# haskoin/haskoin-node

Measured on AMD Instinct MI355X. Metric: ECDSA verifies/sec (1/8 GPU) + verdict mismatches vs libsecp256k1, higher is better.
Workload: dtype u32 (256-bit integer limbs)

## Files before the change

haskoin-node_amd/csrc/hkv_group.h:

```cpp
#pragma once
#include "hkv_scalar.h"

namespace hkv {

struct ge { fe x, y; };
struct gej { fe x, y, z; };


__constant__ static const uint32_t FE_GX[8] = {0x16F81798u, 0x59F2815Bu, 0x2DCE28D9u, 0x029BFCDBu,
                                               0xCE870B07u, 0x55A06295u, 0xF9DCBBACu, 0x79BE667Eu};
__constant__ static const uint32_t FE_GY[8] = {0xFB10D4B8u, 0x9C47D08Fu, 0xA6855419u, 0xFD17B448u,
                                               0x0E1108A8u, 0x5DA4FBFCu, 0x26A3C465u, 0x483ADA77u};
__constant__ static const uint32_t FE_BETA[8] = {0x719501EEu, 0xC1396C28u, 0x12F58995u, 0x9CF04975u,
                                                 0xAC3434E9u, 0x6E64479Eu, 0x657C0710u, 0x7AE96A2Bu};

HKV_DEV void ge_set_g(ge& r) {
#pragma unroll
  for (int i = 0; i < 8; ++i) { r.x.v[i] = FE_GX[i]; r.y.v[i] = FE_GY[i]; }
}
HKV_DEV void gej_set_ge(gej& r, const ge& a) {
  r.x = a.x;
  r.y = a.y;
  fe_set_u32(r.z, 1);
}
HKV_DEV void gej_cmov(gej& r, const gej& a, bool f) {
  fe_cmov(r.x, a.x, f);
  fe_cmov(r.y, a.y, f);
  fe_cmov(r.z, a.z, f);
}

template <bool FC = false>
HKV_DEV void gej_double(gej& r, const gej& a) {
  fe A, B, M, E, t, u;
  fe_sqr<FC>(A, a.x);
  fe_sqr<FC>(B, a.y);
  fe_mul<FC>(M, a.x, B);
  fe_mul_small(E, A, 3);
  fe_half(E, E);
  fe_mul<FC>(r.z, a.y, a.z);
  fe_sqr<FC>(t, E);
  fe_shl(u, M, 1);
  fe_sub(r.x, t, u);
  fe_sub(t, r.x, M);
  fe_sqrmul_sum<FC>(t, B, E, t);
  fe_neg_compl(r.y, t);
}

template <bool FC = false>
HKV_DEV void gej_add_tail(gej& r, const gej& a, const fe& h, const fe& rr) {
  fe hh, hhh, v, t, t2;
  fe_sqr<FC>(hh, h);
  fe_mul<FC>(hhh, h, hh);
  fe_mul<FC>(v, a.x, hh);
  fe_mul<FC>(r.z, a.z, h);
  fe_sqr<FC>(t, rr);
  fe_sub(t, t, hhh);
  fe_shl(t2, v, 1);
  fe_sub(r.x, t, t2);
  fe_sub(v, r.x, v);
  fe_mul_sum<FC>(v, rr, v, a.y, hhh);
  fe_neg_compl(r.y, v);
}

template <bool FC = false>
HKV_DEV void gej_add_ge_core(gej& r, const gej& a, const fe& az, const fe& bx, const fe& by,
                             bool& hz, bool& rz, fe* zr) {
  fe z2, u2, s2, h, rr, t;
  fe_sqr<FC>(z2, az);
  fe_mul<FC>(u2, bx, z2);
  fe_mul<FC>(t, az, z2);
  fe_mul<FC>(s2, by, t);
  fe_sub(h, u2, a.x);
  fe_sub(rr, s2, a.y);
  hz = fe_is_zero(h);
  rz = fe_is_zero(rr);
  gej_add_tail<FC>(r, a, h, rr);
  if (zr) *zr = h;
}

template <bool FC = false>
HKV_DEV void gej_accumulate(gej& acc, bool& inf, const fe& az, const fe& tx, const fe& ty, bool take) {
  fe h, rr;
  {
    fe z2, t;
    fe_sqr<FC>(z2, az);
    fe_mul<FC>(h, tx, z2);
    fe_mul<FC>(t, az, z2);
    fe_mul<FC>(rr, ty, t);
  }
  fe_sub(h, h, acc.x);
  fe_sub(rr, rr, acc.y);
  const bool live = take && !inf;
  const bool hz = fe_is_zero(h);
  if (live && !hz) gej_add_tail<FC>(acc, acc, h, rr);
  const bool degen = live && hz;
  if (__builtin_expect(__any(degen), 0)) {
    const bool rz = fe_is_zero(rr);
    if (degen && rz) gej_double<FC>(acc, acc);
    inf = inf || (degen && !rz);
  }
}
HKV_DEV void gej_double_ilp(gej& r, const gej& a) {
  fe A, B, M, Z3, C, E, t;
  fe_sqr2(A, a.x, B, a.y);
  fe_mul2(M, a.x, B, Z3, a.y, a.z);
  fe_mul_small(E, A, 3);
  fe_half(E, E);
  fe_sqr2(C, B, t, E);
  r.z = Z3;
  fe_shl(B, M, 1);
  fe_sub(r.x, t, B);
  fe_sub(t, M, r.x);
  fe_mul(t, E, t);
  fe_sub(r.y, t, C);
}

HKV_DEV void gej_accumulate_ilp(gej& acc, bool& inf, const fe& az, const fe& tx, const fe& ty, bool take) {
  fe h, rr, hh;
  {
    fe z2, t;
    fe_sqr(z2, az);
    fe_mul2(h, tx, z2, t, az, z2);
    fe_sub(h, h, acc.x);
    fe_sqrmul(hh, h, rr, ty, t);
  }
  fe_sub(rr, rr, acc.y);
  const bool live = take && !inf;
  const bool hz = fe_is_zero(h);
  if (live && !hz) {
    fe hhh, v, r2, z3, t2;
    fe_mul2(hhh, h, hh, v, acc.x, hh);
    fe_sqrmul(r2, rr, z3, acc.z, h);
    acc.z = z3;
    fe_sub(r2, r2, hhh);
    fe_shl(t2, v, 1);
    fe_sub(acc.x, r2, t2);
    fe_sub(v, v, acc.x);
    fe_mul2(v, rr, v, hhh, acc.y, hhh);
    fe_sub(acc.y, v, hhh);
  }
  const bool degen = live && hz;
  if (__builtin_expect(__any(degen), 0)) {
    const bool rz = fe_is_zero(rr);
    if (degen && rz) gej_double(acc, acc);
    inf = inf || (degen && !rz);
  }
}

HKV_DEV uint32_t dpp_xch(uint32_t v) {
  return (uint32_t)__builtin_amdgcn_mov_dpp((int)v, 0xB1, 0xF, 0xF, false);
}
HKV_DEV uint32_t dpp_bc1(uint32_t v) {
  return (uint32_t)__builtin_amdgcn_mov_dpp((int)v, 0xF5, 0xF, 0xF, false);
}
HKV_DEV uint32_t dpp_bc0(uint32_t v) {
  return (uint32_t)__builtin_amdgcn_mov_dpp((int)v, 0xA0, 0xF, 0xF, false);
}
HKV_DEV void fe_xch(fe& r, const fe& a) {
#pragma unroll
  for (int i = 0; i < 8; ++i) r.v[i] = dpp_xch(a.v[i]);
}
HKV_DEV void fe_bc1(fe& r, const fe& a) {
#pragma unroll
  for (int i = 0; i < 8; ++i) r.v[i] = dpp_bc1(a.v[i]);
}
HKV_DEV void fe_sel(fe& r, const fe& a, const fe& b, uint32_t odd) {
#pragma unroll
  for (int i = 0; i < 8; ++i) r.v[i] = (a.v[i] & ~odd) | (b.v[i] & odd);
}
HKV_DEV bool pair_even(bool f) { return dpp_bc0(f ? 1u : 0u) != 0; }
HKV_DEV bool pair_odd(bool f) { return dpp_bc1(f ? 1u : 0u) != 0; }

HKV_DEV void pair_double(fe& P, fe& Z, uint32_t odd) {
  fe R1, T, O1, R2, R3, P1, P2, r, Q, t;
  fe_sqr(R1, P);
  fe_xch(T, R1);
  fe_sel(O1, T, Z, odd);
  fe_mul(R2, P, O1);
  fe_sqr(R3, T);
  fe_sel(P2, R2, R3, odd);
  fe_xch(P1, P2);
  fe_sel(O1, R3, R2, odd);
  fe_lin2(r, P1, odd ? 36u : 9u, P2, odd ? 27u : 8u);
  fe_shl_var(Q, O1, odd ? 1u : 3u);
  fe_xch(O1, Q);
  fe_cneg(O1, O1, odd != 0);
  fe_mul_add(t, T, r, O1);
  fe_sel(P, r, t, odd);
  Z = Q;
}

HKV_DEV void pair_add_tail(fe& P, fe& Z, const fe& H, const fe& R3, const fe& Rr, uint32_t odd) {
  fe O1, O2, R5, R6, W, X3, D, R7, t;
  fe_sel(O1, H, Rr, odd);
  fe_sel(O2, R3, Rr, odd);
  fe_mul(R5, O1, O2);
  fe_xch(t, H);
  fe_sel(O1, P, Z, odd);
  fe_sel(O2, R3, t, odd);
  fe_mul(R6, O1, O2);
  fe_xch(W, R5);
  fe_sub(X3, W, R5);
  fe_shl(t, R6, 1);
  fe_sub(X3, X3, t);
  fe_sub(D, R6, X3);
  fe_xch(t, D);
  fe_xch(O1, P);
  fe_sel(O1, O1, Rr, odd);
  fe_sel(O2, R5, t, odd);
  fe_mul(R7, O1, O2);
  fe_xch(t, R7);
  fe_sub(t, R7, t);
  fe_sel(P, X3, t, odd);
  Z = R6;
}

HKV_DEV void pair_accumulate(fe& P, fe& Z, bool& inf, const fe& TXY, bool take, uint32_t odd) {
  fe z2, O1, O2, R2, H, R3, Rr;
  fe_sqr(z2, Z);
  fe_bc1(O2, z2);
  fe_sel(O1, TXY, Z, odd);
  fe_mul(R2, O1, O2);
  fe_sub(H, R2, P);
  fe_sel(O1, H, TXY, odd);
  fe_sel(O2, H, R2, odd);
  fe_mul(R3, O1, O2);
  fe_sub(Rr, R3, P);
  const bool live = take && !inf;
  const bool hz = pair_even(fe_is_zero(H));
  if (live && !hz) pair_add_tail(P, Z, H, R3, Rr, odd);
// ... 135 lines not shown
```

haskoin-node_amd/csrc/hkv_kernels.hip:

```cpp
#include "hkv_group.h"
#include "hkv_hash.h"
#include "hkv_layout.h"
#include "hkv_joint_digits.h"
#include "hkv_internal.h"
#include "hkv_sighash_dev.h"
#include "hkv_tail_plan.h"

namespace hkv {

HKV_DEV uint32_t rec_word_at(const uint32_t* w, int off) {
  const int k = off >> 2, s = off & 3;
  if (s == 0) return w[k];
  return __builtin_amdgcn_alignbyte(w[k + 1], w[k], s);
}
HKV_DEV void rec_be256(uint32_t out[8], const uint32_t* w, int off) {
#pragma unroll
  for (int j = 0; j < 8; ++j) out[7 - j] = __builtin_bswap32(rec_word_at(w, off + 4 * j));
}

__constant__ static const uint32_t PMN[8] = {0x2FC9BAEEu, 0x402DA172u, 0x50B75FC4u, 0x45512319u, 1u, 0, 0, 0};

template <class W>
struct SoA {
  W* p;
// ... 361 lines not shown
}

struct StdArgs {
  const uint8_t* txs;
  uint32_t n_tx;
  const uint32_t* txt;
  const uint8_t* scripts;
  uint32_t scripts_len;
  const hkv_input_job* jobs;
  int32_t forkid;
  uint32_t* ms_desc;
  uint64_t* ms_off;
  unsigned long long* ms_ctr;
  const uint32_t* tx_off;
};
HKV_DEV void std_lane_prologue(uint32_t i, uint32_t n, SoAView iv, const StdArgs& sa);

HKV_DEV uint4* qtab_ptr(uint32_t* qs, uint32_t n_lanes, uint32_t lane, int entry, int c) {
  return reinterpret_cast<uint4*>(qs) + ((size_t)entry * n_lanes + lane) * QTAB_QUADS_PER_ENTRY + c;
}
HKV_DEV void qtab_store(uint32_t* __restrict__ qs, uint32_t n_lanes, uint32_t lane, int entry, int c, const fe& a) {
  uint4* p = qtab_ptr(qs, n_lanes, lane, entry, c);
  p[0] = make_uint4(a.v[0], a.v[1], a.v[2], a.v[3]);
  p[1] = make_uint4(a.v[4], a.v[5], a.v[6], a.v[7]);
}
HKV_DEV void qtab_load(const uint32_t* __restrict__ qs, uint32_t n_lanes, uint32_t lane, int entry, int c, fe& a) {
  const uint4* p = qtab_ptr(const_cast<uint32_t*>(qs), n_lanes, lane, entry, c);
  const uint4 v0 = p[0], v1 = p[1];
  a.v[0] = v0.x; a.v[1] = v0.y; a.v[2] = v0.z; a.v[3] = v0.w;
  a.v[4] = v1.x; a.v[5] = v1.y; a.v[6] = v1.z; a.v[7] = v1.w;
}

template <bool ILP>
HKV_DEV void ec_double(gej& acc) {
  if constexpr (ILP) gej_double_ilp(acc, acc);
  else gej_double<true>(acc, acc);
}
template <bool ILP>
HKV_DEV void ec_accumulate(gej& acc, bool& inf, const fe& az, const fe& tx, const fe& ty, bool take) {
  if constexpr (ILP) gej_accumulate_ilp(acc, inf, az, tx, ty, take);
  else gej_accumulate<true>(acc, inf, az, tx, ty, take);
}

template <bool ILP = false>
HKV_DEV void gsum_lane(SoACView iv, const uint32_t* __restrict__ gtab, uint32_t i, bool valid, gej& A, bool& ainf);
HKV_DEV void gej_add_var(gej& acc, bool& inf, const gej& b, bool binf);
HKV_DEV bool x_matches_r(const fe& Xin, const fe& Z, const uint32_t r[8]);

HKV_DEV void lane_q(ge& q, SoACView iv, uint32_t i, bool valid) {
  fe x, w;
#pragma unroll
  for (int k = 0; k < 8; ++k) {
    x.v[k] = iv.get(IM_QX, k, i);
    w.v[k] = iv.get(IM_W, k, i);
  }
  fe_mul(q.x, x, w);
  fe_sqr(q.y, w);
  if (!valid) ge_set_g(q);
}

HKV_DEV void qtable_build(const ge& q, uint32_t* __restrict__ qs, uint32_t n_lanes, uint32_t lane, fe& Zg) {
  gej p2, pj;
  gej_set_ge(p2, q);
  gej_double(p2, p2);
  fe z2, qx, qy;
  fe_sqr(z2, p2.z);
  fe_mul(qx, q.x, z2);
  fe_mul(z2, z2, p2.z);
  fe_mul(qy, q.y, z2);
  qtab_store(qs, n_lanes, lane, 0, 0, qx);
  qtab_store(qs, n_lanes, lane, 0, 2, qy);
  qtab_store(qs, n_lanes, lane, 1, 0, p2.x);
  qtab_store(qs, n_lanes, lane, 1, 2, p2.y);
  pj.x = p2.x;
  pj.y = p2.y;
  fe_set_u32(pj.z, 1);
#pragma unroll 1
  for (int j = 2; j < QTAB_ENTRIES; ++j) {
    bool hz, rz;
    fe h;
    gej_add_ge_core(pj, pj, pj.z, qx, qy, hz, rz, &h);
    qtab_store(qs, n_lanes, lane, j, 0, pj.x);
    qtab_store(qs, n_lanes, lane, j, 2, pj.y);
    qtab_store(qs, n_lanes, lane, (j - 1), 4, h);
  }
  fe_mul(Zg, p2.z, pj.z);
  fe beta;
#pragma unroll
  for (int k = 0; k < 8; ++k) beta.v[k] = FE_BETA[k];
  {
    fe bx;
    fe_mul(bx, pj.x, beta);
    qtab_store(qs, n_lanes, lane, QTAB_ENTRIES - 1, 4, bx);
  }
  fe rho;
  fe_set_u32(rho, 1);
#pragma unroll 1
  for (int j = QTAB_ENTRIES - 2; j >= 0; --j) {
    fe x, y, t;
    if (j >= 1) {
      qtab_load(qs, n_lanes, lane, j, 4, t);
      fe_mul(rho, rho, t);
    }
    qtab_load(qs, n_lanes, lane, j, 0, x);
    qtab_load(qs, n_lanes, lane, j, 2, y);
    fe_sqr(t, rho);
    fe_mul(x, x, t);
    fe_mul(t, t, rho);
    fe_mul(y, y, t);
    qtab_store(qs, n_lanes, lane, j, 0, x);
    qtab_store(qs, n_lanes, lane, j, 2, y);
    fe_mul(x, x, beta);
    qtab_store(qs, n_lanes, lane, j, 4, x);
  }
}

typedef uint32_t JqLds[4][8][WG];
HKV_DEV uint4* jq_ptr(uint32_t* qs, uint32_t n_lanes, uint32_t lane, int entry, int c) {
  return reinterpret_cast<uint4*>(qs) + ((size_t)entry * n_lanes + lane) * JQ_QUADS_PER_ENTRY + c;
}
HKV_DEV void quads_store(uint4* p, const fe& a) {
  p[0] = make_uint4(a.v[0], a.v[1], a.v[2], a.v[3]);
  p[1] = make_uint4(a.v[4], a.v[5], a.v[6], a.v[7]);
}
HKV_DEV void quads_load(const uint4* p, fe& a) {
  const uint4 v0 = p[0], v1 = p[1];
  a.v[0] = v0.x; a.v[1] = v0.y; a.v[2] = v0.z; a.v[3] = v0.w;
  a.v[4] = v1.x; a.v[5] = v1.y; a.v[6] = v1.z; a.v[7] = v1.w;
}
HKV_DEV void jq_load(const uint32_t* __restrict__ qs, uint32_t n_lanes, uint32_t lane, int entry, int c, fe& a) {
  quads_load(jq_ptr(const_cast<uint32_t*>(qs), n_lanes, lane, entry, c), a);
}
struct JqPark {
  JqLds* lds;
  uint4 *spare, *zslot, *last;
  HKV_DEV uint4* quads(int h) const { return h < 6 ? spare + 2 * (h - 4) : h == 6 ? zslot : last + 2 * (h - 7); }
  HKV_DEV void store(int h, const fe& a) const {
    if (h < 4) {
#pragma unroll
      for (int k = 0; k < 8; ++k) (*lds)[h][k][threadIdx.x] = a.v[k];
    } else {
      quads_store(quads(h), a);
    }
  }
  HKV_DEV void load(int h, fe& a) const {
    if (h < 4) {
#pragma unroll
      for (int k = 0; k < 8; ++k) a.v[k] = (*lds)[h][k][threadIdx.x];
    } else {
      quads_load(quads(h), a);
    }
  }
};
HKV_DEV void qtable_build_joint(const ge& q, uint32_t* __restrict__ qs, uint32_t n_lanes, uint32_t lane, uint4* zslot,
                                JqLds* lds, fe& Zg) {
  static_assert(JD_ENTRIES == JQ_ENTRIES, "one entry per orbit");
  const JqPark park = {lds, reinterpret_cast<uint4*>(qs) + (size_t)JQ_ENTRIES * JQ_QUADS_PER_ENTRY * n_lanes +
                                (size_t)lane * JQ_SPARE_QUADS,
                       zslot, jq_ptr(qs, n_lanes, lane, JQ_ENTRIES - 1, 0)};
  gej p2, pj;
  gej_set_ge(p2, q);
  gej_double(p2, p2);
  {
    fe z2, qx, qy;
    fe_sqr(z2, p2.z);
    fe_mul(qx, q.x, z2);
    fe_mul(z2, z2, p2.z);
    fe_mul(qy, q.y, z2);
    quads_store(jq_ptr(qs, n_lanes, lane, 0, 0), qx);
    quads_store(jq_ptr(qs, n_lanes, lane, 0, 2), qy);
  }
  quads_store(jq_ptr(qs, n_lanes, lane, 1, 0), p2.x);
  quads_store(jq_ptr(qs, n_lanes, lane, 1, 2), p2.y);
  pj.x = p2.x;
  pj.y = p2.y;
  fe_set_u32(pj.z, 1);
#pragma unroll 1
  for (int j = 2; j < JQ_ENTRIES; ++j) {
    const uint32_t e = (JD_STEP_E >> (2 * (j - 1))) & 3u;
    const bool neg = ((JD_STEP_S >> (j - 1)) & 1u) != 0;
    bool hz, rz;
    fe h, tx, ty;
    jq_load(qs, n_lanes, lane, 0, 0, tx);
    if (e != 0u) {
      fe beta, bx;
#pragma unroll
      for (int k = 0; k < 8; ++k) beta.v[k] = FE_BETA[k];
      fe_mul(bx, tx, beta);
      if (e == 2u) {
        fe_add(bx, tx, bx);
        fe_neg(bx, bx);
      }
      tx = bx;
    }
    jq_load(qs, n_lanes, lane, 0, 2, ty);
    fe_cneg(ty, ty, neg);
    gej_add_ge_core(pj, pj, pj.z, tx, ty, hz, rz, &h);
    if (j < JQ_ENTRIES - 1) {
      quads_store(jq_ptr(qs, n_lanes, lane, j, 0), pj.x);
      quads_store(jq_ptr(qs, n_lanes, lane, j, 2), pj.y);
    }
    park.store(j - 2, h);
  }
  fe_mul(Zg, p2.z, pj.z);
  fe rho;
  fe_set_u32(rho, 1);
#pragma unroll 1
  for (int j = JQ_ENTRIES - 2; j >= 0; --j) {
    fe x, y, t;
    if (j >= 1) {
      park.load(j - 1, t);
      fe_mul(rho, rho, t);
    }
    jq_load(qs, n_lanes, lane, j, 0, x);
    jq_load(qs, n_lanes, lane, j, 2, y);
    fe_sqr(t, rho);
    fe_mul(x, x, t);
    fe_mul(t, t, rho);
    fe_mul(y, y, t);
    quads_store(jq_ptr(qs, n_lanes, lane, j, 0), x);
    quads_store(jq_ptr(qs, n_lanes, lane, j, 2), y);
  }
  quads_store(park.last, pj.x);
  quads_store(park.last + 2, pj.y);
}

template <bool ILP>
HKV_DEV void q_chain(gej& acc, bool& inf, SoACView iv, uint32_t i, bool valid, const uint32_t* __restrict__ qs,
                     uint32_t n_lanes, uint32_t lane, const uint32_t& signs) {
  inf = true;
  fe_set_zero(acc.x);
  fe_set_zero(acc.y);
  fe_set_zero(acc.z);
  uint32_t dw = valid ? iv.get(IM_DIG, NWIN - 1, i) : DIG_ZERO;
  int win = NWIN - 1;
  bool dbl = false;
  int x1 = 0, x2 = 0;
  int nterm = 2;
  {
    const uint32_t dw2 = valid ? iv.get(IM_DIG, NWIN - 2, i) : DIG_ZERO;
    const int t1 = (((int)(dw & QDIG_MASK) - QBIAS) << QW) + (int)(dw2 & QDIG_MASK) - QBIAS;
    const int t2 = (((int)((dw >> QDIG_BITS) & QDIG_MASK) - QBIAS) << QW) + (int)((dw2 >> QDIG_BITS) & QDIG_MASK) - QBIAS;
    if (!__any(t1 < 0 || t1 > 2 * QBIAS || t2 < 0 || t2 > 2 * QBIAS)) {
      const int e1 = t1 < QBIAS ? t1 : QBIAS, e2 = t2 < QBIAS ? t2 : QBIAS;
      x1 = t1 - e1;
      x2 = t2 - e2;
      dw = (uint32_t)(e1 + QBIAS) | ((uint32_t)(e2 + QBIAS) << QDIG_BITS);
      win = NWIN - 2;
      nterm = 4;
    }
  }
#pragma unroll 1
  for (; win >= 0; --win) {
    const int d1 = (int)(dw & QDIG_MASK) - QBIAS, d2 = (int)((dw >> QDIG_BITS) & QDIG_MASK) - QBIAS;
    const uint32_t dw_next = (win > 0 && valid) ? iv.get(IM_DIG, win - 1, i) : DIG_ZERO;
    if (dbl) {
#pragma unroll 1
      for (int d = 0; d < QW; ++d) {
        if (!inf) ec_double<ILP>(acc);
      }
    }
    dbl = true;
#pragma unroll 1
    for (int t = 0; t < nterm; ++t) {
      const int slot = t & 1;
      const int dg = t < 2 ? (slot == 0 ? d1 : d2) : (slot == 0 ? x1 : x2);
      const bool take = dg != 0;
      if (t >= 2 && !__any(take)) continue;
      const int mg = dg < 0 ? -dg : dg;
      const int ie = mg ? mg - 1 : 0;
      const bool neg = (dg < 0) != (((signs >> slot) & 1u) != 0);
      fe tx, ty;
      qtab_load(qs, n_lanes, lane, ie, (slot == 0 ? 0 : 4), tx);
      qtab_load(qs, n_lanes, lane, ie, 2, ty);
      fe_cneg(ty, ty, neg);
      const bool was_inf = inf;
      ec_accumulate<ILP>(acc, inf, acc.z, tx, ty, take);
      if (__any(take && was_inf)) gej_accumulate_from_inf(acc, inf, tx, ty, take && was_inf);
    }
    nterm = 2;
    dw = dw_next;
  }
}

template <class DigitWord>
HKV_DEV void joint_digits_lane(uint32_t (*jd)[WG], uint32_t signs, DigitWord word) {
  constexpr uint32_t QM = (1u << QW) - 1u;
  uint32_t k1[5] = {0, 0, 0, 0, 0}, k2[5] = {0, 0, 0, 0, 0};
  int c1 = 0, c2 = 0;
#pragma unroll
  for (int w = 0; w < NWIN; ++w) {
    const uint32_t dw = word(w);
    const int t1 = (int)(dw & QDIG_MASK) - QBIAS + c1, t2 = (int)((dw >> QDIG_BITS) & QDIG_MASK) - QBIAS + c2;
    const uint32_t n1 = (uint32_t)t1 & QM, n2 = (uint32_t)t2 & QM;
    c1 = (t1 - (int)n1) >> QW;
    c2 = (t2 - (int)n2) >> QW;
    const int q = (QW * w) >> 5, sh = (QW * w) & 31;
    k1[q] |= n1 << sh;
    k2[q] |= n2 << sh;
    if (sh + QW > 32 && q < 4) {
      k1[q + 1] |= n1 >> (32 - sh);
      k2[q + 1] |= n2 >> (32 - sh);
    }
  }
  jd_signed(k1, (signs & 1u) != 0);
  jd_signed(k2, (signs & 2u) != 0);
  uint32_t out[JD_WORDS];
  joint_recode(k1, k2, out);
#pragma unroll
  for (int q = 0; q < JD_WORDS; ++q) jd[q][threadIdx.x] = out[q];
}
HKV_DEV void q_chain_joint(gej& acc, bool& inf, const uint32_t (*jd)[WG], const uint32_t* __restrict__ qs,
                           uint32_t n_lanes, uint32_t lane) {
  inf = true;
  fe_set_zero(acc.x);
  fe_set_zero(acc.y);
  fe_set_zero(acc.z);
  int win = JD_WINDOWS - 1;
#pragma unroll 1
  while (win > 0 && !__any(((jd[win >> 2][threadIdx.x] >> (7 * (win & 3))) & JD_ENTRY_MASK) != JD_ZERO)) --win;
  bool dbl = false;
#pragma unroll 1
  for (; win >= 0; --win) {
    const uint32_t code = (jd[win >> 2][threadIdx.x] >> (7 * (win & 3))) & JD_CODE_MASK;
    const uint32_t ent = code & JD_ENTRY_MASK;
    const bool take = ent != JD_ZERO;
    if (dbl) {
#pragma unroll 1
      for (int d = 0; d < 3; ++d) {
        if (!inf) ec_double<false>(acc);
      }
    }
    dbl = true;
    const int ie = take ? (int)ent : 0;
    const uint32_t e = (code >> JD_E_SHIFT) & 3u;
    const bool e2 = take && e == 2u;
    fe tx, ty;
    jq_load(qs, n_lanes, lane, ie, 0, tx);
    const bool e1 = take && e == 1u;
    if (__any(e1 || e2)) {
      fe beta, bx;
#pragma unroll
      for (int k = 0; k < 8; ++k) beta.v[k] = FE_BETA[k];
      fe_mul<true>(bx, tx, beta);
      fe_cmov(tx, bx, e1);
      fe_add(bx, tx, bx);
      fe_cmov(tx, bx, e2);
      fe_cneg(tx, tx, e2);
    }
    jq_load(qs, n_lanes, lane, ie, 2, ty);
    fe_cneg(ty, ty, (code >> JD_S_SHIFT) != 0u);
    const bool was_inf = inf;
    ec_accumulate<false>(acc, inf, acc.z, tx, ty, take);
    if (__any(take && was_inf)) gej_accumulate_from_inf(acc, inf, tx, ty, take && was_inf);
  }
}

HKV_DEV void clock_probe(unsigned long long* __restrict__ clk, int slot) {
  if (clk != nullptr && blockIdx.x == 0 && threadIdx.x == 0) {
    clk[slot] = clock64();
    clk[slot + 1] = wall_clock64();
  }
}

template <bool ILP, bool STDPRO = false>
__global__ void __launch_bounds__(WG, 2) hkv_ecmult_kernel(uint32_t* __restrict__ im, uint32_t n, uint32_t n_pad,
                                                           uint32_t* __restrict__ qs,
                                                           unsigned long long* __restrict__ clk, StdArgs sa) {
  static_assert(ILP, "only the paired-form (mid-size) instance is built: larger batches run 2a");
  const uint32_t n_lanes = gridDim.x * WG;
  const uint32_t lane = blockIdx.x * WG + threadIdx.x;
  __shared__ uint32_t park[9][WG];
  clock_probe(clk, 0);

  for (uint32_t base = blockIdx.x * WG; base < n_pad; base += gridDim.x * WG) {
    const uint32_t i = base + threadIdx.x;
    if constexpr (STDPRO) std_lane_prologue(i, n, SoAView{im, n_pad}, sa);
// ... 1577 lines not shown
      const bool okk = ecmult_simple(o, u, zero, g);
      for (int k = 0; k < 8; ++k) { res[k] = o.x.v[k]; res[8 + k] = o.y.v[k]; }
      if (!okk) res[15] ^= 0xFFFFFFFFu;
      break;
    }
    case HKV_DBG_MUL512: mul512(res, x.v, y.v); break;
    case HKV_DBG_SQR512: sqr512(res, x.v); break;
    case HKV_DBG_FE_CNEG: fe_cneg(z, x, (y.v[0] & 1u) != 0); raw_norm(z); break;
    case HKV_DBG_FE_CNEG_MASK: fe_cneg_mask(z, x, 0u - (y.v[0] & 1u)); raw_norm(z); break;
    case HKV_DBG_FE_NEG: fe_neg(z, x); raw_norm(z); break;
    case HKV_DBG_FE_HALF: fe_half(z, x); raw_norm(z); break;
    case HKV_DBG_FE_SHL: {
      const uint32_t s = y.v[0];
      if (s == 1u) fe_shl(z, x, 1);
      else fe_shl(z, x, (int)s);
      raw_norm(z);
      break;
    }
    case HKV_DBG_FE_SHL_VAR: fe_shl_var(z, x, y.v[0]); raw_norm(z); break;
    case HKV_DBG_FE_MUL_SMALL: fe_mul_small(z, x, y.v[0]); raw_norm(z); break;
    case HKV_DBG_FE_MUL_SMALL2: {
      fe xn, z2;
      load_next(xn, a);
      fe_mul_small2(z, x, y.v[0], z2, xn, y.v[1]);
      norm_pair(z, z2);
      break;
    }
    case HKV_DBG_FE_LIN2: {
      const uint32_t kk = b[inext * 8];
      fe_lin2(z, x, kk & 0xFFu, y, (kk >> 8) & 0xFFu);
      raw_norm(z);
      break;
    }
    case HKV_DBG_FE_MUL_ADD: {
      fe xn;
      load_next(xn, a);
      fe_mul_add<true>(z, x, y, xn);
      raw_norm(z);
      break;
    }
    case HKV_DBG_FE_MUL2: {
      fe xn, yn, z2;
      load_next(xn, a);
      load_next(yn, b);
      fe_mul2(z, x, y, z2, xn, yn);
      norm_pair(z, z2);
      break;
    }
    case HKV_DBG_FE_SQR2: {
      fe z2;
      fe_sqr2(z, x, z2, y);
      norm_pair(z, z2);
      break;
    }
    case HKV_DBG_FE_SQRMUL: {
      fe xn, z2;
      load_next(xn, a);
      fe_sqrmul(z, x, z2, y, xn);
      norm_pair(z, z2);
      break;
    }
    case HKV_DBG_FE_MUL_REF: fe_mul_ref(z, x, y); raw_norm(z); break;
    case HKV_DBG_FE_SQR_REF: fe_sqr_ref(z, x); raw_norm(z); break;
    case HKV_DBG_FE_NORMALIZE: z = x; fe_normalize(z); for (int k = 0; k < 8; ++k) res[k] = z.v[k]; break;
    case HKV_DBG_FE_IS_ZERO: res[0] = fe_is_zero(x) ? 1u : 0u; break;
    case HKV_DBG_FE_EQUAL: res[0] = fe_equal(x, y) ? 1u : 0u; break;
    case HKV_DBG_U256_LT_P: res[0] = u256_lt_p(x.v) ? 1u : 0u; break;
    case HKV_DBG_SC_ADD: sc_add(wres, u, v); for (int k = 0; k < 8; ++k) res[k] = wres.v[k]; break;
    case HKV_DBG_SC_SUB: sc_sub(wres, u, v); for (int k = 0; k < 8; ++k) res[k] = wres.v[k]; break;
    case HKV_DBG_SC_NEG: sc_neg(wres, u); for (int k = 0; k < 8; ++k) res[k] = wres.v[k]; break;
    case HKV_DBG_SC_SQR: sc_sqr(wres, u); for (int k = 0; k < 8; ++k) res[k] = wres.v[k]; break;
    case HKV_DBG_SC_IS_HIGH: res[0] = sc_is_high(u) ? 1u : 0u; break;
    case HKV_DBG_INV_MOD_P: sgcd::inv_mod_p(res, x.v); break;
    case HKV_DBG_FE_MUL_SUM:
    case HKV_DBG_FE_MUL_SUM_RA:
    case HKV_DBG_FE_MUL_SUM_RB:
    case HKV_DBG_FE_MUL_SUM_RD: {
      fe xn, yn;
      load_next(xn, a);
      load_next(yn, b);
      if (op == HKV_DBG_FE_MUL_SUM_RA) { fe_mul_sum<true>(x, x, y, xn, yn); z = x; }
      else if (op == HKV_DBG_FE_MUL_SUM_RB) { fe_mul_sum<true>(y, x, y, xn, yn); z = y; }
      else if (op == HKV_DBG_FE_MUL_SUM_RD) { fe_mul_sum<true>(yn, x, y, xn, yn); z = yn; }
      else fe_mul_sum<true>(z, x, y, xn, yn);
      raw_norm(z);
      break;
    }
    case HKV_DBG_FE_SQRMUL_SUM:
    case HKV_DBG_FE_SQRMUL_SUM_RA:
    case HKV_DBG_FE_SQRMUL_SUM_RD: {
      fe xn;
      load_next(xn, a);
      if (op == HKV_DBG_FE_SQRMUL_SUM_RA) { fe_sqrmul_sum<true>(x, x, y, xn); z = x; }
      else if (op == HKV_DBG_FE_SQRMUL_SUM_RD) { fe_sqrmul_sum<true>(xn, x, y, xn); z = xn; }
      else fe_sqrmul_sum<true>(z, x, y, xn);
      raw_norm(z);
      break;
    }
    case HKV_DBG_FE_NEG_COMPL: fe_neg_compl(z, x); raw_norm(z); break;
    case HKV_DBG_FC_MUL:
    case HKV_DBG_FC_SQR:
    case HKV_DBG_FC_MUL_ADD:
    case HKV_DBG_FC_MUL_SUM:
    case HKV_DBG_FC_SQRMUL_SUM:
    case HKV_DBG_FC_MUL_MASK: {
      fe xn, yn;
      load_next(xn, a);
      load_next(yn, b);
      uint64_t T = 0, rare;
      if (op == HKV_DBG_FC_SQR) rare = sqr256_red_ps_fc(z.v, T, x.v, x.v);
      else if (op == HKV_DBG_FC_MUL_ADD) rare = mul256_red_add_ps_fc(z.v, T, x.v, y.v, xn.v);
      else if (op == HKV_DBG_FC_MUL_SUM) rare = mul256_red_sum_ps_fc(z.v, T, x.v, y.v, xn.v, yn.v);
      else if (op == HKV_DBG_FC_SQRMUL_SUM) rare = sqrmul256_red_sum_ps_fc(z.v, T, x.v, y.v, xn.v);
      else rare = mul256_red_ps_fc(z.v, T, x.v, y.v);
      if (op == HKV_DBG_FC_MUL_MASK) {
        res[0] = (uint32_t)rare;
        res[1] = (uint32_t)(rare >> 32);
        break;
      }
      for (int k = 0; k < 8; ++k) res[k] = z.v[k];
      res[8] = (uint32_t)T;
      res[9] = (uint32_t)(T >> 32);
      res[10] = (uint32_t)(rare >> (threadIdx.x & 63u)) & 1u;
      break;
    }
    case HKV_DBG_JOINT_RECODE: {
      __shared__ uint32_t jd[JD_WORDS][WG];
      uint32_t S1[5], S2[5], dig[NWIN];
      for (int k = 0; k < 5; ++k) { S1[k] = x.v[k]; S2[k] = y.v[k]; }
      uint32_t p1 = 0, p2 = 0;
#pragma unroll
      for (int w = 0; w < NWIN; ++w) {
        constexpr uint32_t QM = (1u << QW) - 1u;
        const uint32_t v1 = p1 | ((S1[0] & QM) << 1), v2 = p2 | ((S2[0] & QM) << 1);
        p1 = (S1[0] >> (QW - 1)) & 1u;
        p2 = (S2[0] >> (QW - 1)) & 1u;
        shr_bits<5>(S1, QW);
        shr_bits<5>(S2, QW);
        const int d1 = (int)((v1 + 1u) >> 1) - (int)((v1 >> QW) << QW);
        const int d2 = (int)((v2 + 1u) >> 1) - (int)((v2 >> QW) << QW);
        dig[w] = (uint32_t)(d1 + QBIAS) | ((uint32_t)(d2 + QBIAS) << QDIG_BITS);
      }
      joint_digits_lane(jd, (x.v[5] & 1u) | ((y.v[5] & 1u) << 1), [&](int w) { return dig[w]; });
      for (int k = 0; k < JD_WORDS; ++k) res[k] = jd[k][threadIdx.x];
      break;
    }
    case HKV_DBG_JOINT_TABLE: {
      __shared__ JqLds park;
      uint32_t tab[(QTAB_QUADS + QTAB_ZG_QUADS) * 4];
      ge g, q;
      sc zero;
      for (int k = 0; k < 8; ++k) zero.v[k] = 0;
      ge_set_g(g);
      if (!ecmult_simple(q, u, zero, g)) q = g;
      fe Zg, zi, zi2, t;
      qtable_build_joint(q, tab, 1u, 0u, reinterpret_cast<uint4*>(tab) + QTAB_QUADS, &park, Zg);
      const int j = (int)(y.v[0] & 15u) < JD_ENTRIES ? (int)(y.v[0] & 15u) : 0;
      jq_load(tab, 1u, 0u, j, 0, x);
      jq_load(tab, 1u, 0u, j, 2, z);
      fe_inv(zi, Zg);
      fe_sqr(zi2, zi);
      fe_mul(x, x, zi2);
      fe_mul(t, zi2, zi);
      fe_mul(z, z, t);
      norm_pair(x, z);
      break;
    }
    default: break;
  }
#pragma unroll
  for (int k = 0; k < 16; ++k) out[i * 16 + k] = res[k];
}

__global__ void __launch_bounds__(WG) hkv_debug_group_kernel(uint32_t op, uint32_t lanes,
                                                             const uint32_t* __restrict__ a,
                                                             const uint32_t* __restrict__ b,
                                                             uint32_t* __restrict__ out) {
  const uint32_t i = blockIdx.x * WG + threadIdx.x;
  if (i >= lanes) return;
  sc k1, k2, zero;
  fe z1, w;
#pragma unroll
  for (int k = 0; k < 8; ++k) {
    k1.v[k] = a[(2 * i) * 8 + k];
    z1.v[k] = a[(2 * i + 1) * 8 + k];
    k2.v[k] = b[(2 * i) * 8 + k];
    w.v[k] = b[(2 * i + 1) * 8 + k];
    zero.v[k] = 0;
  }
  const uint32_t sel = w.v[0];
  const bool take = (sel & 1u) != 0;
  ge g, p1, p2, o;
  ge_set_g(g);
  fe_set_zero(o.x);
  fe_set_zero(o.y);
  bool oinf = false;
  uint32_t flag = 0;
  if (op == HKV_DBG_X_MATCHES_R) {
    fe X, zz, xin;
#pragma unroll
    for (int k = 0; k < 8; ++k) xin.v[k] = k1.v[k];
    fe_sqr(zz, z1);
    fe_mul(X, xin, zz);
    o.x.v[0] = x_matches_r(X, z1, k2.v) ? 1u : 0u;
  } else if (op == HKV_DBG_ECMULT) {
    sc kp;
#pragma unroll
    for (int k = 0; k < 8; ++k) kp.v[k] = z1.v[k];
    p1 = g;
    const bool pok = ecmult_simple(p2, kp, zero, g);
    if (!pok) p2 = g;
    oinf = !ecmult_simple(p1, k1, k2, p2);
    if (!oinf) o = p1;
  } else {
    p1 = g;
    p2 = g;
    ge t;
    const bool ok1 = ecmult_simple(t, k1, zero, g);
    if (ok1) p1 = t;
    const bool ok2 = ecmult_simple(t, k2, zero, g);
    if (ok2) p2 = t;
    gej acc;
    fe zz, zzz;
    fe_sqr(zz, z1);
    fe_mul(zzz, zz, z1);
    fe_mul(acc.x, p1.x, zz);
    fe_mul(acc.y, p1.y, zzz);
    acc.z = z1;
    bool inf = !ok1 || (sel & 2u) != 0;
    switch (op) {
      case HKV_DBG_GEJ_DOUBLE: gej_double<true>(acc, acc); break;
      case HKV_DBG_GEJ_DOUBLE_ILP: gej_double_ilp(acc, acc); break;
      case HKV_DBG_GEJ_ACCUMULATE: gej_accumulate<true>(acc, inf, acc.z, p2.x, p2.y, take); break;
      case HKV_DBG_GEJ_ACCUMULATE_ILP: gej_accumulate_ilp(acc, inf, acc.z, p2.x, p2.y, take); break;
      case HKV_DBG_GEJ_ADD_AFFINE_COMPLETE: gej_add_affine_complete(acc, inf, p2, take); break;
      case HKV_DBG_GEJ_ADD_VAR: {
        gej bj;
        fe_sqr(zz, w);
        fe_mul(zzz, zz, w);
        fe_mul(bj.x, p2.x, zz);
        fe_mul(bj.y, p2.y, zzz);
        bj.z = w;
        gej_add_var(acc, inf, bj, !ok2 || (sel & 4u) != 0);
        break;
      }
      default: break;
    }
    oinf = inf;
    if (!inf) {
      fe zi, zi2, zi3;
      fe_inv(zi, acc.z);
      fe_sqr(zi2, zi);
      fe_mul(zi3, zi2, zi);
      fe_mul(o.x, acc.x, zi2);
      fe_mul(o.y, acc.y, zi3);
      fe_normalize(o.x);
      fe_normalize(o.y);
    }
  }
  flag = oinf ? 1u : 0u;
#pragma unroll
  for (int k = 0; k < 8; ++k) {
    out[(2 * i) * 16 + k] = oinf ? 0u : o.x.v[k];
    out[(2 * i) * 16 + 8 + k] = oinf ? 0u : o.y.v[k];
  }
  out[(2 * i + 1) * 16] = flag;
#pragma unroll
  for (int k = 1; k < 16; ++k) out[(2 * i + 1) * 16 + k] = 0;
}

}

namespace hkv {

enum : uint32_t { TQ_CLAIM = 0, TQ_DONE = 1, TQ_SLOT = 8 };
HKV_DEV bool tail_wait(const MsTail& a, unsigned int* done, uint32_t want) {
  uint32_t spins = 0;
  while (a.force_fault || __hip_atomic_load(done, __ATOMIC_ACQUIRE, __HIP_MEMORY_SCOPE_AGENT) < want) {
    if (a.force_fault || spins++ >= (1u << 24)) {
      atomicOr(a.fault, 1u);
      if (a.status) atomicOr(a.status, (uint32_t)HKV_STATUS_TAIL_FAULT);
      return false;
    }
    __builtin_amdgcn_s_sleep(8);
  }
  return true;
}
HKV_DEV void publish_count(unsigned int* ctr) {
  __builtin_amdgcn_s_waitcnt(0);
  __syncthreads();
  if (threadIdx.x == 0) __hip_atomic_fetch_add(ctr, 1u, __ATOMIC_RELEASE, __HIP_MEMORY_SCOPE_AGENT);
}

__global__ void __launch_bounds__(PAIR_TPB, 1) hkv_ms_tail_kernel(MsTail a) {
  __shared__ QLane qlds[2];
  __shared__ HLane hlds[2];
  __shared__ uint32_t xch[25 * PAIR_SIGS];
  __shared__ uint32_t buf[16 * PAIR_TPB];
  __shared__ TailItem item_s;
  __shared__ uint32_t go_s;
  unsigned int* q = a.bar + (a.epoch & 1u) * TQ_SLOT;
  if (blockIdx.x == 0 && threadIdx.x == 0) {
    unsigned int* nx = a.bar + ((a.epoch + 1u) & 1u) * TQ_SLOT;
#pragma unroll
    for (int k = 0; k < (int)TQ_SLOT; ++k) __hip_atomic_store(&nx[k], 0u, __ATOMIC_RELAXED, __HIP_MEMORY_SCOPE_AGENT);
    __hip_atomic_store(a.total_next, 0ull, __ATOMIC_RELAXED, __HIP_MEMORY_SCOPE_AGENT);
  }
  const unsigned long long total = __hip_atomic_load(a.total, __ATOMIC_RELAXED, __HIP_MEMORY_SCOPE_AGENT);
  const uint32_t n_cand = (uint32_t)total, n_keys = (uint32_t)(total >> 32);
// ... 216 lines not shown
```

Baseline: 149.8 million.

## Build joint Q table with co-Z additions sharing the doubled point's Z

Replaces the mixed Jacobian additions in the per-signature Q-table build with co-Z (ZADDU) additions, updating the base point's coordinates in place so each step needs fewer field multiplications. The running base is rotated by beta powers and re-negated instead of being reloaded from memory, and the back-substitution loop is restructured to fold the Z ratios differently. It also templatizes the field ops on an FC flag and extends the debug path to test arbitrary points and the Zg output. The co-Z formulas have edge-case risks when points coincide, which the new debug hooks are meant to probe.

```diff
diff --git a/haskoin-node_amd/csrc/hkv_group.h b/haskoin-node_amd/csrc/hkv_group.h
--- a/haskoin-node_amd/csrc/hkv_group.h
+++ b/haskoin-node_amd/csrc/hkv_group.h
@@ -76,6 +76,24 @@
   rz = fe_is_zero(rr);
   gej_add_tail<FC>(r, a, h, rr);
   if (zr) *zr = h;
+}
+
+template <bool FC = false>
+HKV_DEV void gej_zaddu(fe& x3, fe& y3, fe& px, fe& py, const fe& rx, const fe& ry, fe& h) {
+  fe c, w2, d, t;
+  fe_sub(h, px, rx);
+  fe_sqr<FC>(c, h);
+  fe_mul<FC>(w2, rx, c);
+  fe_mul<FC>(px, px, c);
+  fe_sub(d, py, ry);
+  fe_sub(t, px, w2);
+  fe_mul<FC>(py, py, t);
+  fe_sqr<FC>(t, d);
+  fe_sub(t, t, px);
+  fe_sub(x3, t, w2);
+  fe_sub(t, px, x3);
+  fe_mul<FC>(t, d, t);
+  fe_sub(y3, t, py);
 }
 
 template <bool FC = false>
diff --git a/haskoin-node_amd/csrc/hkv_kernels.hip b/haskoin-node_amd/csrc/hkv_kernels.hip
--- a/haskoin-node_amd/csrc/hkv_kernels.hip
+++ b/haskoin-node_amd/csrc/hkv_kernels.hip
@@ -537,77 +537,79 @@
     }
   }
 };
+template <bool FC>
+HKV_DEV void fe_mul_beta_pow(fe& a, uint32_t e) {
+  fe beta, b;
+#pragma unroll
+  for (int k = 0; k < 8; ++k) beta.v[k] = FE_BETA[k];
+  fe_mul<FC>(b, a, beta);
+  if (e == 2u) {
+    fe_add(b, a, b);
+    fe_neg(b, b);
+  }
+  a = b;
+}
+#ifndef HKV_QTABLE_FC
+#define HKV_QTABLE_FC 0
+#endif
+template <bool FC = (HKV_QTABLE_FC != 0)>
 HKV_DEV void qtable_build_joint(const ge& q, uint32_t* __restrict__ qs, uint32_t n_lanes, uint32_t lane, uint4* zslot,
                                 JqLds* lds, fe& Zg) {
   static_assert(JD_ENTRIES == JQ_ENTRIES, "one entry per orbit");
   const JqPark park = {lds, reinterpret_cast<uint4*>(qs) + (size_t)JQ_ENTRIES * JQ_QUADS_PER_ENTRY * n_lanes +
                                 (size_t)lane * JQ_SPARE_QUADS,
                        zslot, jq_ptr(qs, n_lanes, lane, JQ_ENTRIES - 1, 0)};
-  gej p2, pj;
+  gej p2;
   gej_set_ge(p2, q);
-  gej_double(p2, p2);
+  gej_double<FC>(p2, p2);
+  fe xq, yq;
   {
-    fe z2, qx, qy;
-    fe_sqr(z2, p2.z);
-    fe_mul(qx, q.x, z2);
-    fe_mul(z2, z2, p2.z);
-    fe_mul(qy, q.y, z2);
-    quads_store(jq_ptr(qs, n_lanes, lane, 0, 0), qx);
-    quads_store(jq_ptr(qs, n_lanes, lane, 0, 2), qy);
+    fe z2;
+    fe_sqr<FC>(z2, p2.z);
+    fe_mul<FC>(xq, q.x, z2);
+    fe_mul<FC>(z2, z2, p2.z);
+    fe_mul<FC>(yq, q.y, z2);
   }
   quads_store(jq_ptr(qs, n_lanes, lane, 1, 0), p2.x);
   quads_store(jq_ptr(qs, n_lanes, lane, 1, 2), p2.y);
-  pj.x = p2.x;
-  pj.y = p2.y;
-  fe_set_u32(pj.z, 1);
 #pragma unroll 1
   for (int j = 2; j < JQ_ENTRIES; ++j) {
     const uint32_t e = (JD_STEP_E >> (2 * (j - 1))) & 3u;
     const bool neg = ((JD_STEP_S >> (j - 1)) & 1u) != 0;
-    bool hz, rz;
-    fe h, tx, ty;
-    jq_load(qs, n_lanes, lane, 0, 0, tx);
-    if (e != 0u) {
-      fe beta, bx;
-#pragma unroll
-      for (int k = 0; k < 8; ++k) beta.v[k] = FE_BETA[k];
-      fe_mul(bx, tx, beta);
-      if (e == 2u) {
-        fe_add(bx, tx, bx);
-        fe_neg(bx, bx);
-      }
-      tx = bx;
-    }
-    jq_load(qs, n_lanes, lane, 0, 2, ty);
-    fe_cneg(ty, ty, neg);
-    gej_add_ge_core(pj, pj, pj.z, tx, ty, hz, rz, &h);
+    fe h;
+    if (e != 0u) fe_mul_beta_pow<FC>(xq, e);
+    fe_cneg(yq, yq, neg);
+    gej_zaddu<FC>(p2.x, p2.y, xq, yq, p2.x, p2.y, h);
+    fe_cneg(yq, yq, neg);
+    if (e != 0u) fe_mul_beta_pow<FC>(xq, 3u - e);
     if (j < JQ_ENTRIES - 1) {
-      quads_store(jq_ptr(qs, n_lanes, lane, j, 0), pj.x);
-      quads_store(jq_ptr(qs, n_lanes, lane, j, 2), pj.y);
+      quads_store(jq_ptr(qs, n_lanes, lane, j, 0), p2.x);
+      quads_store(jq_ptr(qs, n_lanes, lane, j, 2), p2.y);
     }
     park.store(j - 2, h);
   }
-  fe_mul(Zg, p2.z, pj.z);
+  quads_store(jq_ptr(qs, n_lanes, lane, 0, 0), xq);
+  quads_store(jq_ptr(qs, n_lanes, lane, 0, 2), yq);
   fe rho;
-  fe_set_u32(rho, 1);
+  park.load(JQ_ENTRIES - 3, rho);
 #pragma unroll 1
-  for (int j = JQ_ENTRIES - 2; j >= 0; --j) {
+  for (int j = JQ_ENTRIES - 2;; --j) {
     fe x, y, t;
-    if (j >= 1) {
-      park.load(j - 1, t);
-      fe_mul(rho, rho, t);
-    }
     jq_load(qs, n_lanes, lane, j, 0, x);
     jq_load(qs, n_lanes, lane, j, 2, y);
-    fe_sqr(t, rho);
-    fe_mul(x, x, t);
-    fe_mul(t, t, rho);
-    fe_mul(y, y, t);
+    fe_sqr<FC>(t, rho);
+    fe_mul<FC>(x, x, t);
+    fe_mul<FC>(t, t, rho);
+    fe_mul<FC>(y, y, t);
     quads_store(jq_ptr(qs, n_lanes, lane, j, 0), x);
     quads_store(jq_ptr(qs, n_lanes, lane, j, 2), y);
-  }
-  quads_store(park.last, pj.x);
-  quads_store(park.last + 2, pj.y);
+    if (j == 1) break;
+    park.load(j - 2, t);
+    fe_mul<FC>(rho, rho, t);
+  }
+  fe_mul<FC>(Zg, p2.z, rho);
+  quads_store(park.last, p2.x);
+  quads_store(park.last + 2, p2.y);
 }
 
 template <bool ILP>
@@ -2491,9 +2493,24 @@
       sc zero;
       for (int k = 0; k < 8; ++k) zero.v[k] = 0;
       ge_set_g(g);
-      if (!ecmult_simple(q, u, zero, g)) q = g;
+      if (y.v[1] != 0u) {
+        fe w;
+        fe_sqr(w, x);
+        fe_mul(w, w, x);
+        fe_set_u32(z, 7);
+        fe_add(w, w, z);
+        fe_mul(q.x, x, w);
+        fe_sqr(q.y, w);
+      } else if (!ecmult_simple(q, u, zero, g)) {
+        q = g;
+      }
       fe Zg, zi, zi2, t;
       qtable_build_joint(q, tab, 1u, 0u, reinterpret_cast<uint4*>(tab) + QTAB_QUADS, &park, Zg);
+      if ((y.v[0] & 15u) == 15u) {
+        fe_normalize(Zg);
+        for (int k = 0; k < 8; ++k) res[k] = Zg.v[k];
+        break;
+      }
       const int j = (int)(y.v[0] & 15u) < JD_ENTRIES ? (int)(y.v[0] & 15u) : 0;
       jq_load(tab, 1u, 0u, j, 0, x);
       jq_load(tab, 1u, 0u, j, 2, z);
```

After: 153.0 million (median of 6 runs). 1.02x the previous value.
